# flatironinstitute/bayes-kit

Hardware: AMD Instinct MI355X
Metric: leapfrog steps/sec (whole node), D=1024 × 65 536 chains; ESS/sec (higher is better)
Workload: dtype f64; 1 GPU; BASELINE.json configs[2]: ill-conditioned Gaussian D=1024 (lam=logspace(0,4)), HMC L=64 eps=0.006, diag metric of ones, model-opaque gradient op; chains_per_gpu=65536, dims=1024, leapfrog_steps=64, parallelism=chains sharded x1, chain_tile=8192

## Files before the change

### bayes-kit_amd/bayes_kit_amd/hmc.py

```python
from __future__ import annotations

from typing import Optional

import numpy as np
import torch

from . import _lib
from ._engine import LookAhead, ManyChainSampler
from .adapt import TrajectoryAdam, jitter_steps, shrink_estimate
from .diagnostics import EnergyDiagnostics, RunningCovariance, _gather_sum


class TrajectoryObserver:

    def __init__(self, sampler):
        self._s, self._ta = sampler, TrajectoryAdam(sampler._T)
        self._T_hist, self._steps_hist, self._nonfinite = [], [], 0

    def after_draw(self, tot, eps, window_end, last):
        s = self._s
        self._T_hist.append(float(s._T))
        self._steps_hist.append(int(s._steps))
        self._nonfinite += int(tot[4])
        s._T = self._ta.step(float(tot[3]), float(tot[0]), s._steps * eps, eps, s._max_steps)
# ... 23 lines not shown
        chains: Optional[int] = None,
        chain_id0: int = 0,
        path: str = "auto",
        metric_dense=None,
        precond_diag=None,
        trajectory_length: Optional[float] = None,
        max_steps: int = 1024,
        tuning: Optional[dict] = None,
        ops=None,
        **knobs,
    ):
        fuse_builtin, fuse_steps = self._resolve_path(path)
        tn = self._resolve_tuning(tuning, knobs)
        chain_tile, graph = tn.get("chain_tile"), tn.get("graph")
        prefetch_rng, tune_placement = tn.get("prefetch_rng"), tn.get("tune_placement")
        self._stepsize = stepsize
        self._steps = steps
        self._chees = None
        self._prefetch, self._snap = False, None
        self._T, self._jitter_n, self._last_steps = None, 0, None
        self._max_steps = self._check_max_steps(max_steps)
        self._graph_explicit = graph is True
        if trajectory_length is not None:
            self._T, self._steps_fixed = self._check_T(trajectory_length), steps
            if self._graph_explicit:
                raise ValueError("graph=True cannot be combined with trajectory_length: a captured draw bakes `steps` in")
            graph = False
        if precond_diag is not None and (metric_diag is not None or metric_dense is not None):
            raise ValueError("give precond_diag or metric_diag / metric_dense, not both")
        self._setup(model, metric_diag, init, seed, chains, chain_id0, ops)
        self._M = None
        if metric_dense is not None:
            if metric_diag is not None:
                raise ValueError("give metric_diag or metric_dense, not both")
            if not self._batched:
                raise ValueError("metric_dense needs a batched device model")
            self._install_metric_dense(metric_dense)
            fuse_builtin = False
        if precond_diag is not None:
            self._install_precond(precond_diag)
        self._init_graph(graph, prefetch_rng)
        self._graph_built = self._use_graph
        self._fused_draw = (bool(fuse_builtin) and self._batched and self._M is None and hasattr(model, "bk_hmc_draw"))
        if self._pd is not None and not hasattr(model, "bk_hmc_draw_precond"):
            self._fused_draw = False
        self._fused = self._fused_draw
        self._lanes_traj = (bool(fuse_builtin) and self._batched and self._M is None and hasattr(model, "bk_hmc_proposal"))
        self._step_hook = (bool(fuse_steps) and self._batched and self._M is None and hasattr(model, "bk_leapfrog_step"))
        self._traj_hook = (bool(fuse_builtin) and self._step_hook and hasattr(model, "bk_leapfrog_trajectory"))
        self._chain_tile = self._pick_tile(chain_tile)
        self._fused_zt = self._fused_draw and self._rng_kind == _lib.RNG_PHILOX and self._dim >= 32
        D, C, dev = self._dim, self._C, self._ops.device
        f64 = dict(dtype=torch.float64, device=dev)
        self._rho_bufs = [None if self._fused_zt else torch.empty((D, C), **f64)]
        self._theta_p = torch.empty((D, C), **f64)
        self._grad = torch.empty((D, C), **f64)
        self._grad_p = torch.empty((D, C), **f64)
        self._lp = torch.empty(C, **f64)
        self._lp_p = torch.empty(C, **f64)
        self._kin0_bufs = [torch.empty(C, **f64)]
        self._kin1 = torch.empty(C, **f64)
        self._logu_bufs = [torch.empty(C, **f64)]
        self._ret = torch.empty(C, **f64)
        self._mask = torch.empty(C, dtype=torch.uint8, device=dev)
        self._rho_tile = torch.empty(D * self._chain_tile, **f64) if self._chain_tile < C else None
        self._accepted = torch.zeros(1, dtype=torch.int32, device=dev)
        if self._fused_draw:
            self._part = torch.empty(12 * C, **f64)
        if self._fused_zt:
            dp = (D + 7) // 8 * 8
            self._zt_bufs = [torch.empty((C, dp), **f64)]
        if self._M is not None:
            self._mv = torch.empty((D, C), **f64)
            self._mv_rng = torch.empty((D, C), **f64)
        self._have_cache = False
        self._draws = 0
        self._rebind = self._batched and not self._use_graph
        if prefetch_rng is None:
            prefetch_rng = self._batched and self._ops.device.type == "cuda"
        self._prefetch = bool(prefetch_rng) and self._batched and not self._use_graph
        self._pf_kin_stale = False
        if self._prefetch:
            if self._fused_zt:
                self._zt_bufs.append(torch.empty_like(self._zt_bufs[0]))
                self._rho_bufs.append(None)
            else:
                self._rho_bufs.append(torch.empty((D, C), **f64))
            self._kin0_bufs.append(torch.empty(C, **f64))
            self._logu_bufs.append(torch.empty(C, **f64))
            self._ahead = LookAhead(dev)
            if self._fused_zt:
                self._snap = [torch.empty_like(self._rng_state) for _ in range(2)]
            else:
                self._rng_logical = self._rng_state.clone()
        self.placement = None
        if self._wants_placement_tuning(tune_placement) and not self._fused and self._M is None:
            self._tune_placement()

    def _install_metric_dense(self, metric_dense):
        if isinstance(metric_dense, torch.Tensor) and metric_dense.dim() == 1 and self._M is not None:
            v = metric_dense.to(device=self._ops.device, dtype=torch.float64)
            if v.shape[0] != self._dim:
                raise ValueError(f"a diagonal metric needs {self._dim} entries")
            self._M.copy_(torch.diag(v))
            self._M_chol.copy_(torch.diag(torch.sqrt(v)))
            self._M_inv.copy_(torch.diag(1.0 / v))
            return
        Mt = torch.as_tensor(metric_dense, dtype=torch.float64).cpu()
        if tuple(Mt.shape) != (self._dim, self._dim):
            raise ValueError(f"metric_dense must be ({self._dim}, {self._dim})")
        Mt = 0.5 * (Mt + Mt.t())
        dev_ = self._ops.device
        chol = torch.linalg.cholesky(Mt)
        inv = torch.linalg.inv(Mt)
        inv = 0.5 * (inv + inv.t())
        if self._M is None:
            self._M, self._M_chol, self._M_inv = (x.to(dev_).contiguous() for x in (Mt, chol, inv))
        else:
            self._M.copy_(Mt)
            self._M_chol.copy_(chol)
            self._M_inv.copy_(inv)

    def set_metric_dense(self, metric_dense):
        if self._M is None:
            raise ValueError("this sampler was built without metric_dense")
        self._install_metric_dense(metric_dense)
        self._drop_ahead(rewind=False)

    @property
    def metric_dense(self):
        return None if self._M is None else self._M.cpu().numpy().copy()

    def _stream_position(self):
        if self._prefetch and self._ahead.ahead:
            return self._rng_logical if self._snap is None else self._snap[self._ahead.slot]
        return self._rng_state

    def _drop_ahead(self, rewind):
        if self._prefetch and self._ahead.ahead:
            position = self._stream_position()
            self._ahead.drop(wait=True)
            if rewind:
                self._rng_state.copy_(position)

    def _install_precond(self, v):
        if self._M is not None or (self._pd is None and self._metric_dev is not None):
            raise ValueError("precond_diag cannot be combined with metric_diag / metric_dense")
# ... 41 lines not shown
            if self._graph_built and not self._use_graph:
                self._use_graph = True
                self._drop_graphs()
            return
        T = self._check_T(T)
        if self._use_graph:
            if self._graph_explicit:
                raise ValueError("graph=True cannot be combined with trajectory_length: a captured draw bakes `steps` in")
            self._use_graph = False
            self._drop_graphs()
        if self._T is None:
            self._steps_fixed = self._steps
        self._T = T

    @property
    def trajectory_length(self):
        return self._T

    @property
    def max_steps(self):
        return self._max_steps

    @property
    def last_steps(self):
        return self._last_steps

    def _next_steps(self):
        if self._T is not None:
            self._jitter_n += 1
            self._steps = jitter_steps(self._jitter_n, self._T, float(self._stepsize), self._max_steps)
        self._last_steps = int(self._steps)

    def _enter_whole_draw(self):
        self._drop_ahead(rewind=True)
        D, C, dev = self._dim, self._C, self._ops.device
        self._fused_draw = self._fused = True
        self._fused_zt = self._rng_kind == _lib.RNG_PHILOX and D >= 32
        n_slots = 2 if self._prefetch else 1
        if getattr(self, "_part", None) is None:
            self._part = torch.empty(12 * C, dtype=torch.float64, device=dev)
        if self._fused_zt:
            zt = list(getattr(self, "_zt_bufs", []))
            while len(zt) < n_slots:
                zt.append(torch.empty((C, (D + 7) // 8 * 8), dtype=torch.float64, device=dev))
            self._zt_bufs = zt
            self._rho_bufs = [None] * n_slots
            if self._prefetch:
                self._snap = [torch.empty_like(self._rng_state) for _ in range(2)]
        self._pf_kin_stale = False
        self._drop_graphs()

    def _tune_placement(self):
        ops, m, eps = self._ops, self._metric_dev, float(self._stepsize)
        n_rho = len(self._rho_bufs)

        builtin = hasattr(self._model, "bk_eval")

        def cost(a):
            tp, gp, rhos = a[0], a[1], a[2:2 + n_rho]
            ms = sum(self._time_ms(lambda r=r: ops.kick_drift(tp, tp, r, r, gp, m, eps, False, 0.0, True, eps))
                     for r in rhos) / n_rho
            if builtin:
                ms += self._time_ms(lambda: self._model.bk_eval(tp, gp, None))
            return ms

        chosen, rep = self._tune_roles([self._theta_p, self._grad_p] + list(self._rho_bufs) + [self._grad], cost)
        self._theta_p, self._grad_p = chosen[0], chosen[1]
        self._rho_bufs = chosen[2:2 + n_rho]
        self._grad = chosen[2 + n_rho]
        key = "step_ms" if builtin else "kick_drift_ms"
        self.placement = {key + "_as_allocated": rep["ms_as_allocated"], key + "_chosen": rep["ms_chosen"],
                          "assignments_tried": rep["assignments_tried"]}

    _tm_last = False

    @staticmethod
    def tile_major_blocks(C, D, T):
        return [(c0, min(C, c0 + T), D * c0) for c0 in range(0, C, T)]

    def _tm_assemble(self, raw):
        D, C = self._dim, self._C
        flat, out = raw.view(-1), torch.empty((D, C), dtype=raw.dtype, device=raw.device)
        for c0, c1, off in self.tile_major_blocks(C, D, self._chain_tile):
            out[:, c0:c1].copy_(flat[off:off + D * (c1 - c0)].view(D, c1 - c0))
        return out

    @property
    def _theta_p(self):
        return self._tm_assemble(self._thp_raw) if self._tm_last else self._thp_raw

    @_theta_p.setter
    def _theta_p(self, a):
        self._thp_raw = a

    @property
    def _grad_p(self):
        return self._tm_assemble(self._gp_raw) if self._tm_last else self._gp_raw

    @_grad_p.setter
    def _grad_p(self, a):
        self._gp_raw = a

    def _tm_flat(self, name):
        a = getattr(self, name)
        if not a.is_contiguous() or a.numel() != self._dim * self._C:
            a = torch.empty((self._dim, self._C), dtype=a.dtype, device=a.device)
            setattr(self, name, a)
        return a.view(-1)

    def _draw_tile_major(self, th, rho, kin0, logu, g, m, eps, half, L):
        ops, D, C, T = self._ops, self._dim, self._C, self._chain_tile
        thp_f, gp_f = self._tm_flat("_thp_raw"), self._tm_flat("_gp_raw")
        if self._rho_tile is None or self._rho_tile.numel() != D * T:
            self._rho_tile = torch.empty(D * T, dtype=torch.float64, device=ops.device)
        lp0 = self._lp.clone() if self._stat is not None else None
        self._out = torch.empty_like(th) if self._rebind else None
        for c0, c1, off in self.tile_major_blocks(C, D, T):
            n, sl = c1 - c0, slice(c0, c1)
            thp_k, gp_k = thp_f[off:off + D * n].view(D, n), gp_f[off:off + D * n].view(D, n)
            rho_k = self._rho_tile[:D * n].view(D, n)
            gl = None
            for s in range(L):
                if s == 0:
                    ops.kick_drift_ld(th[:, sl], thp_k, rho[:, sl], rho_k, g[:, sl], m, eps, True, -half, True, eps)
                else:
                    ops.kick_drift(thp_k, thp_k, rho_k, rho_k, gl, m, eps, False, 0.0, True, eps)
                gl = self._eval_grad(thp_k, gp_k, self._lp_p[sl] if s == L - 1 else None)
            gl = self._materialize(gl, gp_k)
            if self._pd is not None:
                ops.leapfrog_finish_precond(rho_k, None, gl, self._pd, half, False, self._kin1[sl])
            else:
                ops.leapfrog_finish(rho_k, None, gl, m, half, False, self._kin1[sl])
            if self._energy is not None:
                self._energy.update(self._lp[sl], kin0[sl], self._lp_p[sl], self._kin1[sl], logu[sl], th[:, sl],
                                    chain0=self._chain_id0 + c0)
            ops.mh_accept(_lib.ACCEPT_HMC, self._lp[sl], kin0[sl], self._lp_p[sl], self._kin1[sl], logu[sl],
                          self._mask[sl], self._ret[sl], self._accepted)
            if self._rebind:
                ops.blend_columns_ld(self._mask[sl], th[:, sl], thp_k, self._out[:, sl])
            else:
                ops.select_columns_ld(self._mask[sl], th[:, sl], thp_k)
            ops.select_columns_ld(self._mask[sl], self._grad[:, sl], gp_k)
        if lp0 is not None:
            ops.accept_stat(lp0, kin0, self._lp_p, self._kin1, self._stat, self._stat_work)
        if self._rebind:
            self._theta_dc = self._out
        self._tm_last = True

    LLC_BYTES = 192 << 20
    MIN_TILE = 8192

    @classmethod
    def default_chain_tile(cls, C, D):
        t = cls.LLC_BYTES // (3 * 8 * D)
        t -= t % 2
        return t if t >= cls.MIN_TILE and C >= 2 * t else C

    def _pick_tile(self, chain_tile):
        C = self._C
        if chain_tile is None:
            opaque_loop = (self._batched and self._M is None and hasattr(self._model, "bk_eval")
                           and not self._fused_draw and not self._lanes_traj and not self._step_hook)
            return self.default_chain_tile(C, self._dim) if opaque_loop else C
        t = int(chain_tile)
        return C if t <= 0 or t >= C else max(2, t - t % 2)

    def accept_rate(self) -> float:
        n = self._draws * self._C
        return float(self._accepted.item()) / n if n else float("nan")

    @property
    def last_accept(self):
        return self._mask.bool() if self._batched else bool(self._mask[0].item())

    _energy = None

    def track_energy(self, threshold: float = 1000.0, capture: int = 1024) -> EnergyDiagnostics:
# ... 8 lines not shown
    @property
    def energy(self):
        return self._energy

    def _set_metric(self, m):
        if self._pd is not None:
            raise ValueError("metric_diag cannot be combined with precond_diag")
        super()._set_metric(m)
        self._pf_kin_stale = True

    def _state_tensors(self):
        return {"theta": self._theta_dc, "grad": self._grad, "lp": self._lp, "accepted": self._accepted}

    def _logical_rng(self):
        if self._prefetch and self._ahead.ahead:
            self._ahead.synchronize()
        return self._stream_position()

    def load_state_dict(self, sd):
        if self._prefetch and self._ahead.ahead:
            torch.cuda.synchronize()
        self._drop_ahead(rewind=False)
        if self._rebind:
            self._theta_dc = torch.empty_like(self._theta_dc)
        super().load_state_dict(sd)

    def _state_extra(self):
        return {"stepsize": float(self._stepsize), "precond_diag": self._precond_extra(),
                "trajectory_length": self._T, "max_steps": self._max_steps, "jitter_n": self._jitter_n,
                "metric_dense": None if self._M is None else self._M.cpu().clone()}

    def _load_extra(self, extra):
        if "stepsize" in extra:
            self._stepsize = extra["stepsize"]
        if "trajectory_length" in extra:
            self._max_steps = self._check_max_steps(extra["max_steps"])
            self.set_trajectory_length(extra["trajectory_length"])
            self._jitter_n = int(extra["jitter_n"])
        pv = self._precond_from_extra(extra)
        if pv is not None:
            self.set_precond_diag(pv)
        Md = extra.get("metric_dense")
        if Md is not None:
            if self._M is None:
                raise ValueError("checkpoint holds metric_dense, this sampler was built without one (build it with "
                                 "metric_dense=np.eye(D))")
            self._install_metric_dense(Md)

    def _after_load(self):
        if self._prefetch:
            self._ahead.reset()
        self._pf_kin_stale = False

    def _randomness(self, slot):
        ops = self._ops
        if self._fused_zt:
            ops.normals_chain_major(self._rng_kind, self._rng_state, self._zt_bufs[slot], self._dim,
                                    None if self._snap is None else self._snap[slot])
        elif self._pd is not None:
            ops.momentum_refresh_precond(self._rng_kind, self._rng_state, self._rho_bufs[slot], self._pd,
                                         self._kin0_bufs[slot], self._rng_work)
        elif self._M is None:
            ops.momentum_refresh(self._rng_kind, self._rng_state, None, 0.0, 1.0, self._rho_bufs[slot],
                                 self._metric_dev, None if self._fused_draw else self._kin0_bufs[slot], None,
                                 self._rng_work)
        else:
            ops.momentum_refresh(self._rng_kind, self._rng_state, None, 0.0, 1.0, self._mv_rng, None, None,
                                 None, self._rng_work)
            ops.dense_metric_apply(self._M_chol, self._mv_rng, self._rho_bufs[slot])
            self._dense_kinetic(self._rho_bufs[slot], self._kin0_bufs[slot], self._mv_rng)
        ops.log_uniform(self._rng_kind, self._rng_state, self._logu_bufs[slot])

    def _dense_kinetic(self, rho, kin_out, scratch):
        self._ops.dense_metric_apply(self._M_inv, rho, scratch)
        self._ops.dot_columns(rho, scratch, 0.5, kin_out)

    def _mg(self, g):
        if self._M is None:
            return g
        self._ops.dense_metric_apply(self._M, self._materialize_dense(g), self._mv)
        return self._mv

    def _materialize_dense(self, g):
        if g.dim() == 2 and g.stride(1) == 1:
            return g
        self._ops.relayout(g, self._gp_raw)
        return self._gp_raw

    def _current_randomness(self):
        cur = 0
        if not self._prefetch:
            self._randomness(0)
        else:
            ahead = self._ahead.ahead
            cur = self._ahead.take(self._randomness)
            if self._pf_kin_stale and ahead and not self._fused_draw:
                self._ops.leapfrog_finish(self._rho_bufs[cur], None, None, self._metric_dev, 0.0, False, self._kin0_bufs[cur])
            self._pf_kin_stale = False
            self._ahead.start_next(self._randomness, None if self._snap is not None else (self._rng_logical, self._rng_state))
        self._zt_slot = cur
        return self._rho_bufs[cur], self._kin0_bufs[cur], self._logu_bufs[cur]

    def _graph_key(self):
        return (float(self._stepsize), int(self._steps))

    def _dense_estimator(self, group):
        cov = RunningCovariance(self._dim, self._ops)

        def install(chains_total):
            Mn = shrink_estimate(cov.covariance(group), float(cov.n // self._C) * chains_total)
            self._drop_ahead(rewind=True)
            self.set_metric_dense(Mn)
            cov.reset()

        return (lambda: cov.update(self._theta_dc, layout="dc", group=group)), install

    def warmup(self, draws, target_accept=0.8, adapt_metric=True, group=None, *, adapt_trajectory=False, max_steps=None):
        dense = isinstance(adapt_metric, str)
        if dense:
            if adapt_metric != "dense":
                raise ValueError(f"warmup: adapt_metric must be True, False or 'dense', got {adapt_metric!r}")
            if self._M is None:
                raise ValueError("warmup: adapt_metric='dense' estimates metric_dense and is accepted only on a sampler "
                                 "built with metric_dense= (np.eye(D) is the natural start)")
        elif adapt_metric and (self._M is not None or (self._pd is None and self._metric_dev is not None)):
            raise ValueError("warmup: adapt_metric=True estimates precond_diag, which cannot be combined with "
                             "metric_diag / metric_dense (pass adapt_metric=False to tune the step size alone)")
        if adapt_trajectory:
            if not self._batched:
                raise ValueError("warmup: adapt_trajectory=True needs a batched device model (the gradient is taken across "
                                 "chains)")
            if self._M is not None:
                raise ValueError("warmup: adapt_trajectory=True cannot be combined with metric_dense (the dense velocity is "
                                 "not what the kick and drift kernels hold)")
            if self._graph_explicit:
                raise ValueError("warmup: adapt_trajectory=True jitters every draw, which graph=True cannot replay")
            if max_steps is not None:
                max_steps = self._check_max_steps(max_steps)
        elif max_steps is not None:
            raise ValueError("warmup: max_steps bounds the adapted trajectory, pass it with adapt_trajectory=True")
        draws = self._check_warmup(draws, target_accept)
        observer, was_fused = None, False
        if adapt_trajectory:
            ops, dev, C, D = self._ops, self._ops.device, self._C, self._dim
            if max_steps is not None:
                self._max_steps = max_steps
            self.set_trajectory_length(self._T if self._T is not None else float(self._steps) * float(self._stepsize))
            observer = TrajectoryObserver(self)
            was_fused = self._fused_draw
            if was_fused:
                self._leave_whole_draw()
            sums = torch.zeros(2 * D + 1, dtype=torch.float64, device=dev)
            sums[2 * D] = float(C)
            self._chees = (sums, torch.empty(ops.chees_work_elems(C), dtype=torch.float64, device=dev), group)

        def draw():
            self._next_steps()
            self._draw()
            self._join_ahead()

        metric = (self._dense_estimator if dense else self._diag_estimator) if adapt_metric else None
        try:
            rep = self._warmup_loop(draws, target_accept, group, draw, metric, observer)
        finally:
            self._chees, self._rho_cur = None, None
            self._drop_graphs()
            if was_fused and (self._pd is None or hasattr(self._model, "bk_hmc_draw_precond")):
                self._enter_whole_draw()
        if dense:
            rep["metric_dense"] = self._M.cpu().numpy().copy()
        return rep

    def sample(self):
        self._next_steps()
        self._run_draw(self._draw)
        self._join_ahead()
        self._draws += 1
        return self._draw_out(self._theta_dc, self._ret)

    def _draw(self):
        ops = self._ops
        eps, L, m = float(self._stepsize), int(self._steps), self._metric_dev
        half = 0.5 * eps
        th, thp, gp_raw = self._theta_dc, self._thp_raw, self._gp_raw
        mirror = not self._batched
        self._tm_last = False

        rho, kin0, logu = self._current_randomness()
        chees = self._chees is not None
        self._rho_cur = rho if chees else None

        if self._fused_draw:
            if not self._have_cache:
                self._eval_logp(th, self._lp)
                self._have_cache = True
            zt = self._zt_bufs[self._zt_slot] if self._fused_zt else None
            m_draw = None if (m is None or self._metric_identity) else m
            accept = (self._lp, logu, self._mask, self._ret, self._accepted)
            in_launch = accept if (self._stat is None and self._energy is None) else None
            if self._pd is not None:
                self._model.bk_hmc_draw_precond(th, thp, rho, zt, self._pd, eps, L, self._part, kin0, self._kin1, self._lp_p,
                                                accept=in_launch)
            else:
                self._model.bk_hmc_draw(th, thp, rho, zt, m_draw, eps, L, self._part, kin0, self._kin1, self._lp_p,
                                        accept=in_launch)
            if in_launch is None:
                self._accept(kin0, logu)
            self._take(th, thp)
            return

        if self._lanes_traj and L >= 1 and self._pd is None and not chees:
            if not self._have_cache:
                self._materialize(self._eval_grad(th, self._grad, self._lp), self._grad)
                self._have_cache = True
            if self._model.bk_hmc_proposal(th, rho, self._grad, thp, gp_raw, self._lp_p, self._kin1, m, eps, L):
                self._accept(kin0, logu)
                self._take(th, thp, self._grad, gp_raw)
                return

        if mirror:
            self._eval_logp(th, self._lp)
            g = self._eval_grad(th, self._grad, None)
        else:
            if not self._have_cache:
                self._materialize(self._eval_grad(th, self._grad, self._lp), self._grad)
                self._have_cache = True
            g = self._grad

        if self._M is not None:
            m = None
        if L == 0:
            ops.kick_drift(th, thp, rho, rho, self._mg(g), m, 0.0, True, -half, False, 0.0)
            g_last = g
            if not mirror:
                self._lp_p.copy_(self._lp)
        elif (self._traj_hook and not mirror and self._chain_tile >= self._C
              and self._model.bk_leapfrog_trajectory(th, rho, g, None, thp, rho, gp_raw, self._lp_p, m, eps, L,
                                                     hmc_first=True)):
            self._grad_calls += L
            g_last = gp_raw
        elif (self._chain_tile < self._C and not mirror and self._M is None and not self._step_hook
              and hasattr(ops, "kick_drift_ld") and not chees):
            self._draw_tile_major(th, rho, kin0, logu, g, m, eps, half, L)
            return
        else:
            g_last = None
            T = self._chain_tile
            for c0 in range(0, self._C, T):
                c1 = min(self._C, c0 + T)
                tile = (c0, c1) != (0, self._C)
                v = (lambda a: a[:, c0:c1]) if tile else (lambda a: a)
                th_t, thp_t, rho_t, gp_t, g_t = v(th), v(thp), v(rho), v(gp_raw), v(g)
                lp_t = self._lp_p[c0:c1] if tile else self._lp_p
                gl = None
                for n in range(L):
                    last = n == L - 1
                    if n == 0:
                        ops.kick_drift(th_t, thp_t, rho_t, rho_t, self._mg(g_t), m, eps, True, -half, True, eps)
                    elif self._step_hook and not mirror:
                        self._grad_calls += 1
                        self._model.bk_leapfrog_step(thp_t, rho_t, m, eps)
                    else:
                        ops.kick_drift(thp_t, thp_t, rho_t, rho_t, self._mg(gl), m, eps, False, 0.0, True, eps)
                    if self._step_hook and not mirror and not last:
                        continue
                    want_lp = lp_t if (last and not mirror) else None
                    gl = self._eval_grad(thp_t, gp_t, want_lp)
                if tile:
                    self._materialize(gl, gp_t)
                    g_last = gp_raw
                else:
                    g_last = gl
        if self._pd is not None:
            ops.leapfrog_finish_precond(rho, rho if chees else None, g_last, self._pd, half, False, self._kin1)
        elif self._M is None:
            ops.leapfrog_finish(rho, rho if chees else None, g_last, m, half, False, self._kin1)
        else:
            ops.leapfrog_finish(rho, rho, self._mg(g_last), None, half, False, None)
            self._dense_kinetic(rho, self._kin1, self._mv)
        if mirror:
            self._eval_logp(thp, self._lp_p)
        self._accept(kin0, logu)
        if mirror:
            self._select(self._mask, th, thp)
        else:
            gp = self._materialize(g_last, gp_raw) if L > 0 else None
            self._take(th, thp, self._grad if gp is not None else None, gp)

    def _accept(self, kin0, logu):
        if self._stat is not None:
            self._ops.accept_stat(self._lp, kin0, self._lp_p, self._kin1, self._stat, self._stat_work)
        if self._energy is not None:
            self._energy.update(self._lp, kin0, self._lp_p, self._kin1, logu, self._theta_dc)
        if self._chees is not None:
            self._chees_launch(kin0)
# ... 22 lines not shown
```

### bayes-kit_amd/csrc/bk_integrator.hip

```cpp
#include "bk_common.hpp"
#include "bk_tile_kernels.hpp"

namespace {

constexpr int KD_ROWS = 4;
constexpr int KD_BLOCK = 256;

__device__ __forceinline__ double kd_elem(double th, double rho, double g, double m, bool has_m,
                                          double eps, int use_pre, double pre, int use_kick,
                                          double kick, double& rho_new) {
  double t = has_m ? m * g : g;
  double r = rho;
  if (use_pre) r = r + pre * t;
  if (use_kick) r = r + kick * t;
  rho_new = r;
  return th + eps * r;
}

typedef double dvec2 __attribute__((ext_vector_type(2)));

template <int ROWS, bool NT>
__global__ __launch_bounds__(KD_BLOCK) void k_kick_drift_v2(
    const double* th_in, double* th_out, const double* rho_in, double* rho_out, i64 ld,
    const double* grad, i64 ldg, const double* metric, double eps, int use_pre, double pre,
// ... 709 lines not shown
      k_select_v2<false><<<grid, dim3(256), 0, s>>>(mask, dst0, src0, dst1, src1, nullptr, ld, C / 2, D);
  } else {
    dim3 grid((unsigned)bk_cdiv(C, 256), (unsigned)bk_cdiv(D, SEL_ROWS));
    k_select<<<grid, dim3(256), 0, s>>>(mask, dst0, src0, dst1, src1, copy0, ld, C, D);
  }
  BK_RETURN_LAUNCH_STATUS();
}

int bk_blend_columns(const uint8_t* mask, const double* a, const double* b, double* out, int64_t ld, int64_t C,
                     int64_t D, void* stream) {
  if (!mask || !a || !b || !out || C < 0 || D < 0) return BK_E_ARG;
  if (ld < C) return BK_E_ALIGN;
  if (C == 0 || D == 0) return BK_OK;
  hipStream_t s = bk_stream(stream);
  if (C % 2 == 0 && ld % 2 == 0 && bk_aligned16(a) && bk_aligned16(b) && bk_aligned16(out)) {
    dim3 grid((unsigned)bk_cdiv(C / 2, 256), (unsigned)bk_cdiv(D, SEL_ROWS));
    k_blend_v2<<<grid, dim3(256), 0, s>>>(mask, a, b, out, ld, C / 2, D);
  } else {
    dim3 grid((unsigned)bk_cdiv(C, 256), (unsigned)bk_cdiv(D, SEL_ROWS));
    k_blend<<<grid, dim3(256), 0, s>>>(mask, a, b, out, ld, C, D);
  }
  BK_RETURN_LAUNCH_STATUS();
}

static unsigned ld_rows(i64 n) { return (unsigned)(n < 1 ? 1 : (n > 65535 ? 65535 : n)); }

int bk_leapfrog_kick_drift_ld(const double* theta_in, int64_t ld_ti, double* theta_out, int64_t ld_to,
                              const double* rho_in, int64_t ld_ri, double* rho_out, int64_t ld_ro, const double* grad,
                              int64_t ldg_d, int64_t ldg_c, const double* metric, double eps, int use_pre, double pre,
                              int use_kick, double kick, int64_t C, int64_t D, void* stream) {
  if (!theta_in || !theta_out || !rho_in || !rho_out || !grad || C < 0 || D < 0) return BK_E_ARG;
  if (ld_ti < C || ld_to < C || ld_ri < C || ld_ro < C) return BK_E_ALIGN;
  if ((theta_in == theta_out && ld_ti != ld_to) || (rho_in == rho_out && ld_ri != ld_ro)) return BK_E_ARG;
  if (C == 0 || D == 0) return BK_OK;
  hipStream_t s = bk_stream(stream);
  const bool vec = ldg_c == 1 && C % 2 == 0 && ld_ti % 2 == 0 && ld_to % 2 == 0 && ld_ri % 2 == 0 && ld_ro % 2 == 0 &&
                   ldg_d % 2 == 0 && bk_aligned16(theta_in) && bk_aligned16(theta_out) && bk_aligned16(rho_in) &&
                   bk_aligned16(rho_out) && bk_aligned16(grad);
  if (!vec) {
    dim3 grid((unsigned)bk_cdiv(C, bkt::KDL_BLOCK), ld_rows(D));
    bkt::k_kick_drift_ld_s<<<grid, dim3(bkt::KDL_BLOCK), 0, s>>>(theta_in, ld_ti, theta_out, ld_to, rho_in, ld_ri, rho_out,
                                                                 ld_ro, grad, ldg_d, ldg_c, metric, eps, use_pre, pre,
                                                                 use_kick, kick, C, D);
    BK_RETURN_LAUNCH_STATUS();
  }
  const bool past = bk_streams_past_llc(bk_distinct_arrays({theta_in, theta_out, rho_in, rho_out, grad}) * C * D);
  const bool out_past = bk_streams_past_llc(bk_distinct_arrays({theta_out, rho_out}) * C * D);
  dim3 grid((unsigned)bk_cdiv(C / 2, bkt::KDL_BLOCK), ld_rows(D));
#define BK_KDL_LAUNCH(H)                                                                                              \
  bkt::k_kick_drift_ld<H><<<grid, dim3(bkt::KDL_BLOCK), 0, s>>>(theta_in, ld_ti, theta_out, ld_to, rho_in, ld_ri, rho_out, \
                                                                ld_ro, grad, ldg_d, metric, eps, use_pre, pre, use_kick, \
                                                                kick, C / 2, D)
  if (!past) BK_KDL_LAUNCH(0);
  else if (!out_past) BK_KDL_LAUNCH(bkt::NT_IN);
  else BK_KDL_LAUNCH(bkt::NT_IN | bkt::NT_OUT);
#undef BK_KDL_LAUNCH
  BK_RETURN_LAUNCH_STATUS();
}

int bk_blend_columns_ld(const uint8_t* mask, const double* a, int64_t ld_a, const double* b, int64_t ld_b, double* out,
                        int64_t ld_o, int64_t C, int64_t D, void* stream) {
  if (!mask || !a || !b || !out || C < 0 || D < 0) return BK_E_ARG;
  if (ld_a < C || ld_b < C || ld_o < C) return BK_E_ALIGN;
  if (C == 0 || D == 0) return BK_OK;
  hipStream_t s = bk_stream(stream);
  if (C % 2 == 0 && ld_a % 2 == 0 && ld_b % 2 == 0 && ld_o % 2 == 0 && bk_aligned16(a) && bk_aligned16(b) &&
      bk_aligned16(out)) {
    dim3 grid((unsigned)bk_cdiv(C / 2, 256), ld_rows(bk_cdiv(D, bkt::SELL_ROWS)));
    if (ld_b < ld_a)
      bkt::k_blend_ld<bkt::NT_IN | bkt::NT_OUT><<<grid, dim3(256), 0, s>>>(mask, a, ld_a, b, ld_b, out, ld_o, C / 2, D);
    else
      bkt::k_blend_ld<bkt::NT_IN | bkt::NT_OUT | bkt::NT_TILE><<<grid, dim3(256), 0, s>>>(mask, a, ld_a, b, ld_b, out, ld_o,
                                                                                        C / 2, D);
  } else {
    dim3 grid((unsigned)bk_cdiv(C, 256), ld_rows(D));
    bkt::k_blend_ld_s<<<grid, dim3(256), 0, s>>>(mask, a, ld_a, b, ld_b, out, ld_o, C, D);
  }
  BK_RETURN_LAUNCH_STATUS();
}

int bk_select_columns_ld(const uint8_t* mask, double* dst, int64_t ld_d, const double* src, int64_t ld_s, int64_t C,
                         int64_t D, void* stream) {
  if (!mask || !dst || !src || C < 0 || D < 0) return BK_E_ARG;
  if (ld_d < C || ld_s < C) return BK_E_ALIGN;
  if (C == 0 || D == 0) return BK_OK;
  hipStream_t s = bk_stream(stream);
  if (C % 2 == 0 && ld_d % 2 == 0 && ld_s % 2 == 0 && bk_aligned16(dst) && bk_aligned16(src)) {
    dim3 grid((unsigned)bk_cdiv(C / 2, 256), ld_rows(bk_cdiv(D, bkt::SELL_ROWS)));
    if (ld_s < ld_d)
      bkt::k_select_ld<bkt::NT_IN | bkt::NT_OUT><<<grid, dim3(256), 0, s>>>(mask, dst, ld_d, src, ld_s, C / 2, D);
    else
      bkt::k_select_ld<bkt::NT_IN | bkt::NT_OUT | bkt::NT_TILE><<<grid, dim3(256), 0, s>>>(mask, dst, ld_d, src, ld_s,
                                                                                         C / 2, D);
  } else {
    dim3 grid((unsigned)bk_cdiv(C, 256), ld_rows(D));
    bkt::k_select_ld_s<<<grid, dim3(256), 0, s>>>(mask, dst, ld_d, src, ld_s, C, D);
  }
  BK_RETURN_LAUNCH_STATUS();
}

int bk_mala_logq(const double* theta, const double* grad, const double* theta_prop,
                 const double* grad_prop, int64_t ld, double eps, double* lp_forward,
                 double* lp_reverse, int64_t C, int64_t D, void* stream) {
  if (!theta || !grad || !theta_prop || !grad_prop || !lp_forward || !lp_reverse || C < 0 || D < 0)
    return BK_E_ARG;
  if (ld < C) return BK_E_ALIGN;
// ... 29 lines not shown
```

### bayes-kit_amd/csrc/bk_rng.hip

```cpp
#include "bk_common.hpp"
#include "bk_rng.hpp"
#include "bk_welford.hpp"
#include "ziggurat_tables.inc"

namespace {

__device__ const uint64_t d_zig_ki[256] = BK_ZIG_KI_INIT;
__device__ const uint64_t d_zig_wi[256] = BK_ZIG_WI_BITS_INIT;
__device__ const uint64_t d_zig_fi[256] = BK_ZIG_FI_BITS_INIT;
const uint64_t h_zig_ki[256] = BK_ZIG_KI_INIT;
const uint64_t h_zig_wi[256] = BK_ZIG_WI_BITS_INIT;
const uint64_t h_zig_fi[256] = BK_ZIG_FI_BITS_INIT;

struct ZigLds {
  uint64_t ki[256];
  double wi[256];
  double fi[256];
};

__device__ __forceinline__ void load_tables(ZigLds& t) {
  for (int i = threadIdx.x; i < 256; i += blockDim.x) {
    t.ki[i] = d_zig_ki[i];
    t.wi[i] = bk::u64_as_double(d_zig_wi[i]);
    t.fi[i] = bk::u64_as_double(d_zig_fi[i]);
  }
  __syncthreads();
}

constexpr int RNG_BLOCK = 64;
static inline int rng_block(i64 C) { return C <= 32768 ? 32 : 64; }

__global__ __launch_bounds__(256) void k_init_philox(uint64_t* st, i64 ldr, uint64_t key0,
                                                     uint64_t chain0, i64 C) {
  i64 c = (i64)blockIdx.x * blockDim.x + threadIdx.x;
  if (c >= C) return;
  st[0 * ldr + c] = key0;
  st[1 * ldr + c] = chain0 + (uint64_t)c;
  for (int w = 2; w < 10; ++w) st[w * ldr + c] = 0;
  st[10 * ldr + c] = 4;
}

template <typename G, bool PD = false>
__global__ __launch_bounds__(RNG_BLOCK) void k_refresh(uint64_t* st, i64 ldr, const double* loc_in,
                                                       double loc_mul, double scale, double* out,
                                                       i64 ld, const double* metric, double* kin_out,
                                                       const uint8_t* active, i64 C, i64 D) {
  __shared__ ZigLds tab;
  load_tables(tab);
  i64 c = (i64)blockIdx.x * blockDim.x + threadIdx.x;
  if (c >= C) return;
  if (active && !active[c]) return;
  G g;
  g.load(st, ldr, c);
  const i64 Dq = (D + 3) / 4;
// ... 572 lines not shown
  }
  const int nch = (int)((C - c0 < 64) ? C - c0 : 64);
  if (2 * lane < ldz) {
#pragma unroll 4
    for (int cc = w; cc < nch; cc += 4) {
      const double2 v = *reinterpret_cast<const double2*>(zt + (c0 + cc) * ldz + 2 * lane);
      rk_sm[cc * TS + 2 * lane] = v.x;
      rk_sm[cc * TS + 2 * lane + 1] = v.y;
    }
  }
  __syncthreads();
  const i64 Dq = (D + 3) / 4;
  const i64 dlo = w * Dq, dhi = (dlo + Dq < D) ? dlo + Dq : D;
  double kin = 0.0;
  if (c < C) {
    for (i64 d0 = dlo; d0 < dhi; d0 += 8) {
      double loc[8];
#pragma unroll
      for (int u = 0; u < 8; ++u) loc[u] = (loc_in && d0 + u < dhi) ? loc_in[(d0 + u) * ld + c] : 0.0;
#pragma unroll
      for (int u = 0; u < 8; ++u) {
        if (d0 + u < dhi) {
          double lo = loc_in ? loc[u] * loc_mul : 0.0;
          double v = lo + (PD ? metric[D + d0 + u] : scale) * rk_sm[lane * TS + (int)(d0 + u)];
          out[(d0 + u) * ld + c] = v;
          double mv = PD ? metric[2 * D + d0 + u] * v : (metric ? metric[d0 + u] * v : v);
          kin = kin + v * mv;
        }
      }
    }
  }
  part[w * 64 + lane] = kin;
  __syncthreads();
  if (w != 0 || c >= C) return;
  double s = part[lane];
#pragma unroll
  for (int k = 1; k < 4; ++k) s = s + part[k * 64 + lane];
  const double kc = 0.5 * s;
  kin_out[c] = kc;
  if (BEGIN) {
    b.H[c] = dr_joint(b.logp[c], kc);
    b.h[c] = 0.0;
    const double r0 = 0.0;
    b.rej[c] = r0;
    bk::Philox g;
    g.load(b.state, b.ldr, c);
    double lu = log(bk::next_double(g));
    g.store(b.state, b.ldr, c);
    double retry = b.pr * r0;
    b.alive[c] = (lu < retry) ? 1 : 0;
  }
}

template <bool BEGIN, bool PD = false>
static void refresh_apply_kin_launch(const double* work, i64 dp, const double* loc_in, double loc_mul, double scale,
                                     double* out, i64 ld, const double* metric, double* kin_out, i64 C, i64 D,
                                     const DrBegin& b, hipStream_t s) {
  const size_t lds = (size_t)(64 * (dp + 1) + 256) * sizeof(double);
  if (dp <= 128 && lds <= 65536)
    k_refresh_apply_kin_rows<BEGIN, PD><<<dim3((unsigned)bk_cdiv(C, 64)), dim3(256), lds, s>>>(work, dp, loc_in, loc_mul, scale,
                                                                                          out, ld, metric, kin_out, C, D, b);
  else if (bk_streams_past_llc(bk_distinct_arrays({work, out, loc_in}) * C * D))
    k_refresh_apply_kin<BEGIN, PD, true><<<dim3((unsigned)bk_cdiv(C, 64)), dim3(256), 0, s>>>(work, dp, loc_in, loc_mul, scale,
                                                                                         out, ld, metric, kin_out, C, D, b);
  else
    k_refresh_apply_kin<BEGIN, PD><<<dim3((unsigned)bk_cdiv(C, 64)), dim3(256), 0, s>>>(work, dp, loc_in, loc_mul, scale, out,
                                                                                   ld, metric, kin_out, C, D, b);
}

template <bool PC>
__global__ __launch_bounds__(256) void k_mala_propose_z(const double* th, const double* g, const double* z,
                                                        double* prop, i64 ld, double eps, double s, i64 C, i64 D,
                                                        const double* __restrict__ pc) {
  i64 c = (i64)blockIdx.x * 256 + threadIdx.x;
  i64 d0 = (i64)blockIdx.y * 4;
  if (c >= C) return;
  double a[4], b[4], n[4];
#pragma unroll
  for (int i = 0; i < 4; ++i)
    if (d0 + i < D) {
      i64 o = (d0 + i) * ld + c;
      a[i] = th[o];
      b[i] = g[o];
      n[i] = z[o];
    }
#pragma unroll
  for (int i = 0; i < 4; ++i)
    if (d0 + i < D) {
      if (PC) prop[(d0 + i) * ld + c] = (a[i] + eps * (pc[d0 + i] * b[i])) + s * (pc[D + d0 + i] * n[i]);
      else prop[(d0 + i) * ld + c] = (a[i] + eps * b[i]) + s * n[i];
    }
}

template <bool PC>
__global__ __launch_bounds__(256) void k_mala_propose_zt(const double* th, const double* g, const double* zt,
                                                         i64 ldz, double* prop, i64 ld, double eps, double s,
                                                         i64 C, i64 D, const double* __restrict__ pc) {
  __shared__ double tile[64][65];
  i64 c0 = (i64)blockIdx.x * 64, d0 = (i64)blockIdx.y * 64;
  int tx = threadIdx.x & 63, ty = bk_wave_id();
#pragma unroll 4
  for (int i = 0; i < 16; ++i) {
    int cl = ty + 4 * i;
    i64 cc = c0 + cl, d = d0 + tx;
    tile[cl][tx] = (cc < C && d < D) ? zt[cc * ldz + d] : 0.0;
  }
  __syncthreads();
  i64 cc = c0 + tx;
  if (cc >= C) return;
#pragma unroll 4
  for (int i = 0; i < 16; ++i) {
    int dl = ty + 4 * i;
// ... 371 lines not shown
```

### bayes-kit_amd/csrc/bk_tile_kernels.hpp

```cpp
#pragma once
#include "bk_common.hpp"
#include "bk_mem_policy.hpp"

namespace bkt {

typedef double dvec2 __attribute__((ext_vector_type(2)));

constexpr int NT_IN = 1;
constexpr int NT_OUT = 2;
constexpr int NT_TILE = 4;

template <bool NT, class T>
__device__ __forceinline__ T gload(const T* p) {
  return NT ? __builtin_nontemporal_load(p) : *p;
}
template <bool NT, class T>
__device__ __forceinline__ void gstore(T v, T* p) {
  if (NT) __builtin_nontemporal_store(v, p);
  else *p = v;
}

__device__ __forceinline__ double kd_elem(double th, double rho, double g, double m, bool has_m, double eps, int use_pre,
                                          double pre, int use_kick, double kick, double& rho_new) {
  double t = has_m ? m * g : g;
  double r = rho;
  if (use_pre) r = r + pre * t;
  if (use_kick) r = r + kick * t;
  rho_new = r;
  return th + eps * r;
}

constexpr int KDL_BLOCK = 256;
template <int HINTS>
__global__ __launch_bounds__(KDL_BLOCK) void k_kick_drift_ld(const double* th_in, i64 ld_ti, double* th_out, i64 ld_to,
                                                             const double* rho_in, i64 ld_ri, double* rho_out, i64 ld_ro,
                                                             const double* grad, i64 ldg, const double* metric, double eps,
                                                             int use_pre, double pre, int use_kick, double kick, i64 C2,
                                                             i64 D) {
  constexpr bool NI = (HINTS & NT_IN) != 0, NO = (HINTS & NT_OUT) != 0;
  const i64 c2 = (i64)blockIdx.x * KDL_BLOCK + threadIdx.x;
  if (c2 >= C2) return;
  for (i64 d = blockIdx.y; d < D; d += gridDim.y) {
    const dvec2 t = gload<NI>(reinterpret_cast<const dvec2*>(th_in + d * ld_ti + 2 * c2));
    const dvec2 r = gload<NI>(reinterpret_cast<const dvec2*>(rho_in + d * ld_ri + 2 * c2));
    const dvec2 g = gload<NI>(reinterpret_cast<const dvec2*>(grad + d * ldg + 2 * c2));
    const double m = metric ? metric[d] : 1.0;
    dvec2 rn, tn;
    double rx, ry;
    tn.x = kd_elem(t.x, r.x, g.x, m, metric != nullptr, eps, use_pre, pre, use_kick, kick, rx);
    tn.y = kd_elem(t.y, r.y, g.y, m, metric != nullptr, eps, use_pre, pre, use_kick, kick, ry);
    rn.x = rx;
    rn.y = ry;
    gstore<NO>(rn, reinterpret_cast<dvec2*>(rho_out + d * ld_ro + 2 * c2));
    gstore<NO>(tn, reinterpret_cast<dvec2*>(th_out + d * ld_to + 2 * c2));
  }
}

#define BKT_KD_TILE_POLICY bkm::PLAIN, bkm::SC1, bkm::NT, bkm::PLAIN, bkm::SC1
#define BKT_GRAD_TILE_POLICY bkm::PLAIN, bkm::SC1

template <int PT, int PR, int PG, int ST, int SR>
__global__ __launch_bounds__(KDL_BLOCK) void k_kick_drift_tile(double* th, double* rho, i64 ld, const double* grad, i64 ldg,
                                                               const double* metric, double eps, int use_pre, double pre,
                                                               int use_kick, double kick, i64 C2, i64 D) {
  const i64 c2 = (i64)blockIdx.x * KDL_BLOCK + threadIdx.x, d = blockIdx.y;
  if (c2 >= C2) return;
  const uint32_t bytes = (uint32_t)(16 * C2), c = (uint32_t)c2;
  const bkm::Row rt = {th + d * ld, bytes}, rr = {rho + d * ld, bytes}, rg = {grad + d * ldg, bytes};
  const dvec2 t = bkm::load16<PT>(rt, c), r = bkm::load16<PR>(rr, c), g = bkm::load16<PG>(rg, c);
  const double m = metric ? metric[d] : 1.0;
  dvec2 rn, tn;
  double rx, ry;
  tn.x = kd_elem(t.x, r.x, g.x, m, metric != nullptr, eps, use_pre, pre, use_kick, kick, rx);
  tn.y = kd_elem(t.y, r.y, g.y, m, metric != nullptr, eps, use_pre, pre, use_kick, kick, ry);
  rn.x = rx;
  rn.y = ry;
  bkm::store16<SR>(rn, rr, c);
  bkm::store16<ST>(tn, rt, c);
}

template <int PT, int SG>
__global__ __launch_bounds__(KDL_BLOCK) void k_gauss_grad_tile(const double* th, double* g, i64 ld, const double* lam, i64 C2,
                                                               i64 D) {
  const i64 c2 = (i64)blockIdx.x * KDL_BLOCK + threadIdx.x, d = (i64)gridDim.y - 1 - blockIdx.y;
  if (c2 >= C2) return;
  const uint32_t bytes = (uint32_t)(16 * C2), c = (uint32_t)c2;
  const bkm::Row rt = {th + d * ld, bytes}, rg = {g + d * ld, bytes};
  const dvec2 t = bkm::load16<PT>(rt, c);
  const double l = lam ? lam[d] : 1.0;
  dvec2 o;
  o.x = lam ? -(l * t.x) : -t.x;
  o.y = lam ? -(l * t.y) : -t.y;
  bkm::store16<SG>(o, rg, c);
}

static __global__ __launch_bounds__(KDL_BLOCK) void k_kick_drift_ld_s(const double* th_in, i64 ld_ti, double* th_out, i64 ld_to,
                                                               const double* rho_in, i64 ld_ri, double* rho_out, i64 ld_ro,
// ... 198 lines not shown
      const i64 d = d0 + u * PH + ph;
      if (on && d < dhi) {
        dvec2 v = r[u];
        if (pg) {
          const double tx = metric ? m[u] * g[u].x : g[u].x, ty = metric ? m[u] * g[u].y : g[u].y;
          v.x = r[u].x + half * tx;
          v.y = r[u].y + half * ty;
        }
        if (negate) {
          v.x = -v.x;
          v.y = -v.y;
        }
        if (qr) gstore<NO>(v, reinterpret_cast<dvec2*>(qr + d * ld));
        if (kin_out) {
          const double mx = metric ? km[u] * v.x : v.x, my = metric ? km[u] * v.y : v.y;
          dvec2 tm;
          tm.x = v.x * mx;
          tm.y = v.y * my;
          term[w][u * PH + ph][j] = tm;
        }
      }
    }
    load(d0 + R);
    if (!kin_out) continue;
    __syncthreads();
    if (ph == 0 && on) {
      const i64 left = dhi - d0;
      const int nr = (int)(left < R ? (left < 0 ? 0 : left) : R);
#pragma unroll 8
      for (int i = 0; i < nr; ++i) {
        const dvec2 tm = term[w][i][j];
        kin.x = kin.x + tm.x;
        kin.y = kin.y + tm.y;
      }
    }
    __syncthreads();
  }
  if (!kin_out) return;
  if (ph == 0) part[w][j] = kin;
  __syncthreads();
  if (w == 0 && ph == 0 && on) {
    dvec2 s = part[0][j];
#pragma unroll
    for (int k = 1; k < RED_WAVES; ++k) {
      s.x = s.x + part[k][j].x;
      s.y = s.y + part[k][j].y;
    }
    s.x = 0.5 * s.x;
    s.y = 0.5 * s.y;
    *reinterpret_cast<dvec2*>(kin_out + 2 * c2) = s;
  }
}

}
```

Measured before the change: 123.9 million leapfrog steps/sec.

## Generate momentum per chain tile instead of full-size rho buffers

```diff
diff --git a/bayes-kit_amd/bayes_kit_amd/hmc.py b/bayes-kit_amd/bayes_kit_amd/hmc.py
--- a/bayes-kit_amd/bayes_kit_amd/hmc.py
+++ b/bayes-kit_amd/bayes_kit_amd/hmc.py
@@ -99,7 +99,12 @@
         self._fused_zt = self._fused_draw and self._rng_kind == _lib.RNG_PHILOX and self._dim >= 32
         D, C, dev = self._dim, self._C, self._ops.device
         f64 = dict(dtype=torch.float64, device=dev)
-        self._rho_bufs = [None if self._fused_zt else torch.empty((D, C), **f64)]
+        self._tile_ahead = prefetch_rng is True and self._batched and not self._use_graph
+        lazy = self._tile_rng and not self._use_graph and not self._tile_ahead
+        self._work_dropped = lazy and self._rng_work is not None
+        if lazy:
+            self._rng_work = None
+        self._rho_bufs = [None if (self._fused_zt or lazy) else torch.empty((D, C), **f64)]
         self._theta_p = torch.empty((D, C), **f64)
         self._grad = torch.empty((D, C), **f64)
         self._grad_p = torch.empty((D, C), **f64)
@@ -110,7 +115,7 @@
         self._logu_bufs = [torch.empty(C, **f64)]
         self._ret = torch.empty(C, **f64)
         self._mask = torch.empty(C, dtype=torch.uint8, device=dev)
-        self._rho_tile = torch.empty(D * self._chain_tile, **f64) if self._chain_tile < C else None
+        self._rho_tile, self._tile_work = None, None
         self._accepted = torch.zeros(1, dtype=torch.int32, device=dev)
         if self._fused_draw:
             self._part = torch.empty(12 * C, **f64)
@@ -132,7 +137,7 @@
                 self._zt_bufs.append(torch.empty_like(self._zt_bufs[0]))
                 self._rho_bufs.append(None)
             else:
-                self._rho_bufs.append(torch.empty((D, C), **f64))
+                self._rho_bufs.append(None if lazy else torch.empty((D, C), **f64))
             self._kin0_bufs.append(torch.empty(C, **f64))
             self._logu_bufs.append(torch.empty(C, **f64))
             self._ahead = LookAhead(dev)
@@ -140,6 +145,8 @@
                 self._snap = [torch.empty_like(self._rng_state) for _ in range(2)]
             else:
                 self._rng_logical = self._rng_state.clone()
+        if self._tile_rng:
+            self._tile_workspace()
         self.placement = None
         if self._wants_placement_tuning(tune_placement) and not self._fused and self._M is None:
             self._tune_placement()
@@ -287,21 +294,23 @@
 
     def _tune_placement(self):
         ops, m, eps = self._ops, self._metric_dev, float(self._stepsize)
-        n_rho = len(self._rho_bufs)
+        owned = [r for r in self._rho_bufs if r is not None]
+        n_rho = len(owned)
 
         builtin = hasattr(self._model, "bk_eval")
 
         def cost(a):
-            tp, gp, rhos = a[0], a[1], a[2:2 + n_rho]
+            tp, gp, rhos = a[0], a[1], a[2:2 + n_rho] or [a[2]]
             ms = sum(self._time_ms(lambda r=r: ops.kick_drift(tp, tp, r, r, gp, m, eps, False, 0.0, True, eps))
-                     for r in rhos) / n_rho
+                     for r in rhos) / len(rhos)
             if builtin:
                 ms += self._time_ms(lambda: self._model.bk_eval(tp, gp, None))
             return ms
 
-        chosen, rep = self._tune_roles([self._theta_p, self._grad_p] + list(self._rho_bufs) + [self._grad], cost)
+        chosen, rep = self._tune_roles([self._thp_raw, self._gp_raw] + owned + [self._grad], cost)
         self._theta_p, self._grad_p = chosen[0], chosen[1]
-        self._rho_bufs = chosen[2:2 + n_rho]
+        placed = iter(chosen[2:2 + n_rho])
+        self._rho_bufs = [None if r is None else next(placed) for r in self._rho_bufs]
         self._grad = chosen[2 + n_rho]
         key = "step_ms" if builtin else "kick_drift_ms"
         self.placement = {key + "_as_allocated": rep["ms_as_allocated"], key + "_chosen": rep["ms_chosen"],
@@ -346,18 +355,20 @@
     def _draw_tile_major(self, th, rho, kin0, logu, g, m, eps, half, L):
         ops, D, C, T = self._ops, self._dim, self._C, self._chain_tile
         thp_f, gp_f = self._tm_flat("_thp_raw"), self._tm_flat("_gp_raw")
-        if self._rho_tile is None or self._rho_tile.numel() != D * T:
-            self._rho_tile = torch.empty(D * T, dtype=torch.float64, device=ops.device)
+        self._tile_workspace()
         lp0 = self._lp.clone() if self._stat is not None else None
         self._out = torch.empty_like(th) if self._rebind else None
         for c0, c1, off in self.tile_major_blocks(C, D, T):
             n, sl = c1 - c0, slice(c0, c1)
             thp_k, gp_k = thp_f[off:off + D * n].view(D, n), gp_f[off:off + D * n].view(D, n)
             rho_k = self._rho_tile[:D * n].view(D, n)
+            if rho is None:
+                self._tile_randomness(rho_k, kin0[sl], logu[sl], m, sl)
             gl = None
             for s in range(L):
                 if s == 0:
-                    ops.kick_drift_ld(th[:, sl], thp_k, rho[:, sl], rho_k, g[:, sl], m, eps, True, -half, True, eps)
+                    ops.kick_drift_ld(th[:, sl], thp_k, rho_k if rho is None else rho[:, sl], rho_k, g[:, sl], m, eps, True,
+                                      -half, True, eps)
                 else:
                     ops.kick_drift(thp_k, thp_k, rho_k, rho_k, gl, m, eps, False, 0.0, True, eps)
                 gl = self._eval_grad(thp_k, gp_k, self._lp_p[sl] if s == L - 1 else None)
@@ -472,6 +483,26 @@
             self._ahead.reset()
         self._pf_kin_stale = False
 
+    def _rho_full(self, slot):
+        if self._rho_bufs[slot] is None:
+            self._rho_bufs[slot] = torch.empty((self._dim, self._C), dtype=torch.float64, device=self._ops.device)
+        if self._work_dropped:
+            self._rng_work, self._work_dropped = self._ops.refresh_work(self._C, self._dim), False
+
+    def _tile_workspace(self):
+        D, T, ops = self._dim, self._chain_tile, self._ops
+        if self._rho_tile is None or self._rho_tile.numel() != D * T:
+            self._rho_tile = torch.empty(D * T, dtype=torch.float64, device=ops.device)
+            self._tile_work = ops.refresh_work(T, D) if self._rng_kind == _lib.RNG_PHILOX and D >= 32 else None
+
+    def _tile_randomness(self, rho_k, kin0, logu, m, sl):
+        ops, state = self._ops, self._rng_state[:, sl]
+        if self._pd is not None:
+            ops.momentum_refresh_precond(self._rng_kind, state, rho_k, self._pd, kin0, self._tile_work)
+        else:
+            ops.momentum_refresh(self._rng_kind, state, None, 0.0, 1.0, rho_k, m, kin0, None, self._tile_work)
+        ops.log_uniform(self._rng_kind, state, logu)
+
     def _randomness(self, slot):
         ops = self._ops
         if self._fused_zt:
@@ -509,6 +540,9 @@
 
     def _current_randomness(self):
         cur = 0
+        if not self._fused_zt:
+            for slot in range(len(self._rho_bufs)):
+                self._rho_full(slot)
         if not self._prefetch:
             self._randomness(0)
         else:
@@ -520,6 +554,20 @@
             self._ahead.start_next(self._randomness, None if self._snap is not None else (self._rng_logical, self._rng_state))
         self._zt_slot = cur
         return self._rho_bufs[cur], self._kin0_bufs[cur], self._logu_bufs[cur]
+
+    @property
+    def _tile_rng(self):
+        return (self._chain_tile < self._C and self._batched and self._M is None and not self._step_hook
+                and not self._fused_draw and not self._lanes_traj and hasattr(self._ops, "kick_drift_ld"))
+
+    def _tile_major_draw(self):
+        return self._tile_rng and self._chees is None and int(self._steps) >= 1
+
+    def _tile_major_randomness(self):
+        self._drop_ahead(rewind=True)
+        self._pf_kin_stale = False
+        self._zt_slot = 0
+        return None, self._kin0_bufs[0], self._logu_bufs[0]
 
     def _graph_key(self):
         return (float(self._stepsize), int(self._steps))
@@ -606,7 +654,9 @@
         mirror = not self._batched
         self._tm_last = False
 
-        rho, kin0, logu = self._current_randomness()
+        tiled = self._tile_major_draw()
+        in_line = tiled and not self._tile_ahead
+        rho, kin0, logu = self._tile_major_randomness() if in_line else self._current_randomness()
         chees = self._chees is not None
         self._rho_cur = rho if chees else None
 
@@ -659,8 +709,7 @@
                                                      hmc_first=True)):
             self._grad_calls += L
             g_last = gp_raw
-        elif (self._chain_tile < self._C and not mirror and self._M is None and not self._step_hook
-              and hasattr(ops, "kick_drift_ld") and not chees):
+        elif tiled:
             self._draw_tile_major(th, rho, kin0, logu, g, m, eps, half, L)
             return
         else:
diff --git a/bayes-kit_amd/csrc/bk_integrator.hip b/bayes-kit_amd/csrc/bk_integrator.hip
--- a/bayes-kit_amd/csrc/bk_integrator.hip
+++ b/bayes-kit_amd/csrc/bk_integrator.hip
@@ -785,6 +785,7 @@
                                                                 ld_ro, grad, ldg_d, metric, eps, use_pre, pre, use_kick, \
                                                                 kick, C / 2, D)
   if (!past) BK_KDL_LAUNCH(0);
+  else if (!out_past && rho_in == rho_out) BK_KDL_LAUNCH(bkt::NT_IN | bkt::RHO_PLAIN);
   else if (!out_past) BK_KDL_LAUNCH(bkt::NT_IN);
   else BK_KDL_LAUNCH(bkt::NT_IN | bkt::NT_OUT);
 #undef BK_KDL_LAUNCH
diff --git a/bayes-kit_amd/csrc/bk_rng.hip b/bayes-kit_amd/csrc/bk_rng.hip
--- a/bayes-kit_amd/csrc/bk_rng.hip
+++ b/bayes-kit_amd/csrc/bk_rng.hip
@@ -1,5 +1,6 @@
 #include "bk_common.hpp"
 #include "bk_rng.hpp"
+#include "bk_tile_kernels.hpp"
 #include "bk_welford.hpp"
 #include "ziggurat_tables.inc"
 
@@ -678,12 +679,22 @@
   }
 }
 
+constexpr i64 RK_CUS = 256;
+static bool refresh_tile_shape(const double* work, const double* loc_in, const double* out, i64 ld, const double* kin_out,
+                               i64 C, i64 D) {
+  return C % 2 == 0 && ld % 2 == 0 && bk_aligned16(out) && bk_aligned16(kin_out) && bk_aligned16(loc_in) &&
+         bk_cdiv(C, 64) < RK_CUS && !bk_streams_past_llc(bk_distinct_arrays({work, out, loc_in}) * C * D);
+}
+
 template <bool BEGIN, bool PD = false>
 static void refresh_apply_kin_launch(const double* work, i64 dp, const double* loc_in, double loc_mul, double scale,
                                      double* out, i64 ld, const double* metric, double* kin_out, i64 C, i64 D,
                                      const DrBegin& b, hipStream_t s) {
   const size_t lds = (size_t)(64 * (dp + 1) + 256) * sizeof(double);
-  if (dp <= 128 && lds <= 65536)
+  if (!BEGIN && refresh_tile_shape(work, loc_in, out, ld, kin_out, C, D))
+    bkt::k_refresh_apply_kin_t<8, 8, 0, PD><<<dim3((unsigned)bk_cdiv(C / 2, 8)), dim3(bkt::RED_BLOCK), 0, s>>>(
+        work, dp, loc_in, loc_mul, scale, out, ld, metric, kin_out, C / 2, D);
+  else if (dp <= 128 && lds <= 65536)
     k_refresh_apply_kin_rows<BEGIN, PD><<<dim3((unsigned)bk_cdiv(C, 64)), dim3(256), lds, s>>>(work, dp, loc_in, loc_mul, scale,
                                                                                           out, ld, metric, kin_out, C, D, b);
   else if (bk_streams_past_llc(bk_distinct_arrays({work, out, loc_in}) * C * D))
diff --git a/bayes-kit_amd/csrc/bk_tile_kernels.hpp b/bayes-kit_amd/csrc/bk_tile_kernels.hpp
--- a/bayes-kit_amd/csrc/bk_tile_kernels.hpp
+++ b/bayes-kit_amd/csrc/bk_tile_kernels.hpp
@@ -9,6 +9,7 @@
 constexpr int NT_IN = 1;
 constexpr int NT_OUT = 2;
 constexpr int NT_TILE = 4;
+constexpr int RHO_PLAIN = 8;
 
 template <bool NT, class T>
 __device__ __forceinline__ T gload(const T* p) {
@@ -37,12 +38,12 @@
                                                              const double* grad, i64 ldg, const double* metric, double eps,
                                                              int use_pre, double pre, int use_kick, double kick, i64 C2,
                                                              i64 D) {
-  constexpr bool NI = (HINTS & NT_IN) != 0, NO = (HINTS & NT_OUT) != 0;
+  constexpr bool NI = (HINTS & NT_IN) != 0, NO = (HINTS & NT_OUT) != 0, NR = NI && (HINTS & RHO_PLAIN) == 0;
   const i64 c2 = (i64)blockIdx.x * KDL_BLOCK + threadIdx.x;
   if (c2 >= C2) return;
   for (i64 d = blockIdx.y; d < D; d += gridDim.y) {
     const dvec2 t = gload<NI>(reinterpret_cast<const dvec2*>(th_in + d * ld_ti + 2 * c2));
-    const dvec2 r = gload<NI>(reinterpret_cast<const dvec2*>(rho_in + d * ld_ri + 2 * c2));
+    const dvec2 r = gload<NR>(reinterpret_cast<const dvec2*>(rho_in + d * ld_ri + 2 * c2));
     const dvec2 g = gload<NI>(reinterpret_cast<const dvec2*>(grad + d * ldg + 2 * c2));
     const double m = metric ? metric[d] : 1.0;
     dvec2 rn, tn;
@@ -347,4 +348,93 @@
   }
 }
 
-}
+template <int CP, int U, int HINTS, bool PD>
+__global__ __launch_bounds__(RED_BLOCK) void k_refresh_apply_kin_t(const double* zt, i64 ldz, const double* loc_in,
+                                                                   double loc_mul, double scale, double* out, i64 ld,
+                                                                   const double* metric, double* kin_out, i64 C2, i64 D) {
+  constexpr bool NI = (HINTS & NT_IN) != 0, NO = (HINTS & NT_OUT) != 0;
+  constexpr int PH = BK_WAVE / CP, R = U * PH, NC = 2 * CP;
+  constexpr int TP = NC + 2;
+  static_assert((U & (U - 1)) == 0 && (CP & (CP - 1)) == 0 && CP <= BK_WAVE, "powers of two");
+  __shared__ __attribute__((aligned(16))) double tile[RED_WAVES][R][TP];
+  __shared__ dvec2 part[RED_WAVES][CP];
+  const int lane = threadIdx.x & (BK_WAVE - 1), w = bk_wave_id(), j = lane % CP, ph = lane / CP;
+  const i64 c2 = (i64)blockIdx.x * CP + j, cb = (i64)blockIdx.x * NC, C = 2 * C2;
+  const bool on = c2 < C2;
+  const i64 Dq = (D + RED_WAVES - 1) / RED_WAVES;
+  const i64 dlo = w * Dq, dhi = (dlo + Dq < D) ? dlo + Dq : D;
+  double z[2 * U];
+  auto load = [&](i64 d0) {
+#pragma unroll
+    for (int i = 0; i < 2 * U; ++i) {
+      const int e = i * BK_WAVE + lane;
+      const i64 cc = cb + e / R, d = d0 + e % R;
+      z[i] = (cc < C && d < dhi) ? gload<NI>(zt + cc * ldz + d) : 0.0;
+    }
+  };
+  dvec2 kin = {0.0, 0.0};
+  load(dlo);
+  for (i64 r0 = 0; r0 < Dq; r0 += R) {
+    const i64 d0 = dlo + r0;
+#pragma unroll
+    for (int i = 0; i < 2 * U; ++i) {
+      const int e = i * BK_WAVE + lane;
+      tile[w][e % R][e / R] = z[i];
+    }
+    __syncthreads();
+#pragma unroll
+    for (int u = 0; u < U; ++u) {
+      const int row = u * PH + ph;
+      const i64 d = d0 + row;
+      if (on && d < dhi) {
+        dvec2* cell = reinterpret_cast<dvec2*>(&tile[w][row][2 * j]);
+        const dvec2 zz = *cell;
+        dvec2 lo = {0.0, 0.0};
+        if (loc_in) {
+          const dvec2 l = gload<NO>(reinterpret_cast<const dvec2*>(loc_in + d * ld + 2 * c2));
+          lo.x = l.x * loc_mul;
+          lo.y = l.y * loc_mul;
+        }
+        const double sc = PD ? metric[D + d] : scale;
+        dvec2 v;
+        v.x = lo.x + sc * zz.x;
+        v.y = lo.y + sc * zz.y;
+        gstore<NO>(v, reinterpret_cast<dvec2*>(out + d * ld + 2 * c2));
+        const double m = PD ? metric[2 * D + d] : (metric ? metric[d] : 1.0);
+        const double mx = (PD || metric) ? m * v.x : v.x, my = (PD || metric) ? m * v.y : v.y;
+        dvec2 tm;
+        tm.x = v.x * mx;
+        tm.y = v.y * my;
+        *cell = tm;
+      }
+    }
+    load(d0 + R);
+    __syncthreads();
+    if (ph == 0 && on) {
+      const i64 left = dhi - d0;
+      const int nr = (int)(left < R ? (left < 0 ? 0 : left) : R);
+#pragma unroll 8
+      for (int r = 0; r < nr; ++r) {
+        const dvec2 tm = *reinterpret_cast<const dvec2*>(&tile[w][r][2 * j]);
+        kin.x = kin.x + tm.x;
+        kin.y = kin.y + tm.y;
+      }
+    }
+    __syncthreads();
+  }
+  if (ph == 0) part[w][j] = kin;
+  __syncthreads();
+  if (w == 0 && ph == 0 && on) {
+    dvec2 s = part[0][j];
+#pragma unroll
+    for (int k = 1; k < RED_WAVES; ++k) {
+      s.x = s.x + part[k][j].x;
+      s.y = s.y + part[k][j].y;
+    }
+    s.x = 0.5 * s.x;
+    s.y = 0.5 * s.y;
+    *reinterpret_cast<dvec2*>(kin_out + 2 * c2) = s;
+  }
+}
+
+}
```

New measurement: 126.2 million leapfrog steps/sec (median of 6 runs). 1.9% higher.
